# stanfordnlp/mac-network

Hardware: AMD Instinct MI355X
Metric: questions/sec fwd+bwd (B=64,d=512,p=12,KB=14x14x1024) at 1/2/4/8 MI355X (higher is better)
Workload: dtype f32 (3xfp16-split emulation); 1 GPU

## Files before the change

### mac-network_amd/csrc/macx_wgrad_h2.hip.h

```cpp
#pragma once
#include "macx_gemm_tn.hip.h"
#include "macx_h2.hip.h"

namespace macx {

__device__ __forceinline__ float sum16_h2(float v) {
  v += __shfl_xor(v, 1, 64);
  v += __shfl_xor(v, 2, 64);
  v += __shfl_xor(v, 4, 64);
  v += __shfl_xor(v, 8, 64);
  return v;
}
__device__ __forceinline__ uint32_t pk_mul_f16(uint32_t a, uint32_t b) {
  return __builtin_bit_cast(uint32_t, __builtin_bit_cast(f16x2_t, a) * __builtin_bit_cast(f16x2_t, b));
}
__device__ __forceinline__ uint32_t pk_pow2_f16(int k) {
  const float f = k < -30 ? 0.f : h2_pow2(k);
  return pk_f16(f, f);
}

struct ReadAttBwdH2P {
  int B, N, d;
  const float* att;
  const float* da;
  H2View I2;
  const float* c;
  const float* wk;
  int act;
  const uint8_t* bytes;
  float inv_keep;
  H2View dI2;
  float* dc;
  float* dwk_part;
  float* db2_part;
  float* dbk_part;
  const float* dl;
  int no_out;
};

constexpr int RABH_THREADS = 1024;
constexpr int RABH_CHUNK = 128;
__global__ __launch_bounds__(RABH_THREADS) void read_att_bwd_h2_kernel(ReadAttBwdH2P p) {
  __shared__ float s_dl[1024];
  __shared__ float s_red[RABH_THREADS / 64];
  __shared__ float s_mx[16][RABH_CHUNK];
  const int b = blockIdx.x, slab = blockIdx.y;
  const int tid = threadIdx.x, lane = tid & 63;
  const int wave = __builtin_amdgcn_readfirstlane(tid >> 6);
  constexpr int NWV = RABH_THREADS / 64;
  if (p.dl) {
    for (int n = tid; n < p.N; n += RABH_THREADS) s_dl[n] = p.dl[(size_t)b * p.N + n];
    __syncthreads();
  } else {
  float dot = 0.f;
  for (int n = tid; n < p.N; n += RABH_THREADS) dot += p.att[(size_t)b * p.N + n] * p.da[(size_t)b * p.N + n];
  dot = wave_sum(dot);
  if (lane == 0) s_red[wave] = dot;
  __syncthreads();
  dot = 0.f;
#pragma unroll
  for (int w = 0; w < NWV; ++w) dot += s_red[w];
  __syncthreads();
  float dls = 0.f;
  for (int n = tid; n < p.N; n += RABH_THREADS) {
    const float dl = p.att[(size_t)b * p.N + n] * (p.da[(size_t)b * p.N + n] - dot);
    s_dl[n] = dl;
    dls += dl;
  }
  dls = wave_sum(dls);
  if (lane == 0) s_red[wave] = dls;
  __syncthreads();
  if (tid == 0 && slab == 0) {
    float t = 0.f;
#pragma unroll
    for (int w = 0; w < NWV; ++w) t += s_red[w];
    p.dbk_part[b] = t;
  }
  }

  const int kg = slab * 16 + wave;
  const int col0 = slab * 128 + wave * 8;
  float cv[8], wv[8];
  {
    const f32x4 c0 = *reinterpret_cast<const f32x4*>(p.c + (size_t)b * p.d + col0), c1 = *reinterpret_cast<const f32x4*>(p.c + (size_t)b * p.d + col0 + 4);
    const f32x4 w0 = *reinterpret_cast<const f32x4*>(p.wk + col0), w1 = *reinterpret_cast<const f32x4*>(p.wk + col0 + 4);
#pragma unroll
    for (int e = 0; e < 4; ++e) { cv[e] = c0[e]; cv[4 + e] = c1[e]; wv[e] = w0[e]; wv[4 + e] = w1[e]; }
  }
  const size_t iRp = p.I2.Rp(), oRp = p.dI2.Rp();
  const char* i0 = p.I2.plane(0);
  const size_t ipb = p.I2.plane_bytes(), opb = p.dI2.plane_bytes();
  char* o0 = p.dI2.plane(0);
  const int icb = p.I2.cb(), ocb = p.dI2.cb();
  float a_dc[8], a_dw[8], a_db[8];
#pragma unroll
  for (int e = 0; e < 8; ++e) a_dc[e] = a_dw[e] = a_db[e] = 0.f;

  auto rows = [&](auto act_c) {
    constexpr int ACT = decltype(act_c)::value;
    for (int n0 = 0; n0 < p.N; n0 += RABH_CHUNK) {
      float o[RABH_CHUNK / 64][8];
#pragma unroll
      for (int j = 0; j < RABH_CHUNK / 64; ++j) {
        const int lrow = lane + 64 * j, n = n0 + lrow;
        float m = 0.f;
        if (n < p.N) {
          const size_t row = (size_t)b * p.N + n;
          const char* src = i0 + ((size_t)kg * iRp + row) * 16;
          float i2[8];
          h2_join8(*reinterpret_cast<const u32x4*>(src), *reinterpret_cast<const u32x4*>(src + ipb),
                   h2_pow2(-(int)p.I2.exps()[row * icb + slab]), i2);
          const float dl = s_dl[n];
          const uint32_t bits = p.bytes ? (uint32_t)p.bytes[(size_t)kg * iRp + row] : 0xFFu;
#pragma unroll
          for (int e = 0; e < 8; ++e) {
            const float zv = i2[e] * cv[e];
            const float g = act_apply(ACT, zv);
            const float f = ((bits >> e) & 1u) ? p.inv_keep : 0.f;
            const float dz = (dl * wv[e]) * f * act_grad_from_out(ACT, g);
            const float ov = dz * cv[e];
            o[j][e] = ov;
            a_dw[e] = fmaf(dl, g * f, a_dw[e]);
            a_dc[e] = fmaf(dz, i2[e], a_dc[e]);
            a_db[e] += ov;
            m = fmaxf(m, fabsf(ov));
          }
        }
        s_mx[wave][lrow] = m;
      }
      if (p.no_out) continue;
      __syncthreads();
#pragma unroll
      for (int j = 0; j < RABH_CHUNK / 64; ++j) {
        const int lrow = lane + 64 * j, n = n0 + lrow;
        if (n < p.N) {
          float m = s_mx[0][lrow];
#pragma unroll
          for (int k = 1; k < 16; ++k) m = fmaxf(m, s_mx[k][lrow]);
          const int ex = h2_exponent(m);
          const float sc = h2_pow2(ex);
          float xs[8];
#pragma unroll
          for (int e = 0; e < 8; ++e) xs[e] = o[j][e] * sc;
          u32x4 hi, lo;
          h2_split8(xs, hi, lo);
          const size_t row = (size_t)b * p.N + n;
          char* dst = o0 + ((size_t)kg * oRp + row) * 16;
          *reinterpret_cast<u32x4*>(dst) = hi;
          *reinterpret_cast<u32x4*>(dst + opb) = lo;
          if (wave == 0) p.dI2.exps()[row * ocb + slab] = (int8_t)ex;
        }
      }
      __syncthreads();
    }
  };
  switch (p.act) {
    case ACT_TANH: rows(std::integral_constant<int, ACT_TANH>{}); break;
    case ACT_SIGMOID: rows(std::integral_constant<int, ACT_SIGMOID>{}); break;
    case ACT_ELU: rows(std::integral_constant<int, ACT_ELU>{}); break;
    case ACT_RELU: rows(std::integral_constant<int, ACT_RELU>{}); break;
    default: rows(std::integral_constant<int, ACT_NON>{}); break;
  }
#pragma unroll
  for (int e = 0; e < 8; ++e) {
    a_dc[e] = wave_sum(a_dc[e]);
    a_dw[e] = wave_sum(a_dw[e]);
    a_db[e] = wave_sum(a_db[e]);
  }
  if (lane == 0) {
    float* dc = p.dc + (size_t)b * p.d + col0;
#pragma unroll
    for (int e = 0; e < 8; ++e) {
      dc[e] += a_dc[e];
      p.dwk_part[(size_t)b * p.d + col0 + e] = a_dw[e];
      p.db2_part[(size_t)b * p.d + col0 + e] = a_db[e];
    }
  }
}

struct TnH2P {
  int M;
  int Kd, Jd;
  int nsplit, rows_per_split;
  int R;
  const char* A; size_t a_stride; int a_mod;
  const char* G; size_t g_stride;
  const int* ecomA;
  const int* ecomG;
  int ecom_nb;
  uint16_t* ftab;
  float* part;
  int dbg;
};
__host__ __device__ inline size_t wgrad_h2_mpad(size_t M) { return (M + 63) & ~(size_t)31; }

typedef short s16x4 __attribute__((ext_vector_type(4)));
__device__ __forceinline__ u32x2 tr_read(const char* lds_addr) {
  const s16x4 v = __builtin_amdgcn_ds_read_tr16_b64_v4i16((__attribute__((address_space(3))) s16x4*)lds_addr);
  return __builtin_bit_cast(u32x2, v);
}

constexpr int WH_APL = 8 * 2 * 512;
template <int KW, int JW> constexpr int wh_stage_bytes() { return 2 * (KW + JW) * WH_APL + 256; }
template <int KW, int JW> constexpr int wh_ring() { return KW + JW == 4 ? 2 : (KW + JW == 3 ? 3 : 4); }

__global__ __launch_bounds__(256) void wgrad_h2_factors_kernel(TnH2P p0, TnH2P p1) {
  const TnH2P& p = blockIdx.y ? p1 : p0;
  __shared__ int sE[2][8];
  if (threadIdx.x < 16) {
    const int w = threadIdx.x >> 3, k = threadIdx.x & 7;
    sE[w][k] = h2_emin_final(w ? p.ecomG : p.ecomA, p.ecom_nb, k);
  }
  __syncthreads();
  const size_t mpad = wgrad_h2_mpad((size_t)p.M);
  const size_t m = (size_t)blockIdx.x * 256 + threadIdx.x;
  if (m >= mpad) return;
  const int acb = p.Kd >> 7, gcb = p.Jd >> 7;
  const H2View a0{const_cast<char*>(p.A), p.R, p.Kd}, g0{const_cast<char*>(p.G), p.R, p.Jd};
  if (m >= (size_t)p.M) {
    for (int i = 0; i < acb * gcb; ++i) p.ftab[(size_t)i * mpad + m] = 0;
    return;
  }
  const int ti = (int)(m / p.R), rr = (int)(m - (size_t)ti * p.R);
  const int ar = p.a_mod ? (int)(m % p.a_mod) : rr;
  const int8_t* ea = reinterpret_cast<const int8_t*>(p.A + (p.a_mod ? 0 : (size_t)ti * p.a_stride) + 2 * a0.plane_bytes()) + (size_t)ar * acb;
  const int8_t* eg = reinterpret_cast<const int8_t*>(p.G + (size_t)ti * p.g_stride + 2 * g0.plane_bytes()) + (size_t)rr * gcb;
  for (int k = 0; k < acb; ++k) {
    const int da = sE[0][k] - (int)ea[k];
    for (int j = 0; j < gcb; ++j)
      p.ftab[((size_t)k * gcb + j) * mpad + m] = (uint16_t)(pk_pow2_f16(da + sE[1][j] - (int)eg[j]) & 0xFFFFu);
  }
}

__device__ __forceinline__ void dma4b(const char* g, char* lds_wave_base) {
  const uint32_t l = __builtin_amdgcn_readfirstlane(
      (uint32_t)(uintptr_t)(__attribute__((address_space(3))) char*)lds_wave_base);
  asm volatile("s_mov_b32 m0, %1\n\ts_nop 0\n\tglobal_load_lds_dword %0, off" ::"v"(g), "s"(l) : "memory", "m0");
}

inline int wgrad_pipe_mode() { const int v = tune_get(MACX_TUNE_WGRAD_PIPE, 3); return (v >= 0 && v <= 3) ? v : 3; }

template <int KW, int JW, int PIPE = 0>
__global__ __launch_bounds__(512) void wgrad_h2_kernel(TnH2P p0, TnH2P p1) {
  const TnH2P& p = blockIdx.y ? p1 : p0;
  extern __shared__ __attribute__((aligned(16))) float smem[];
  char* lds = reinterpret_cast<char*>(smem);
  constexpr int KT = KW * T_TILE;
  constexpr int JT = JW * T_TILE;
  constexpr int APL = KW * WH_APL;
  constexpr int GPL = JW * WH_APL;
  constexpr int DATA = 2 * APL + 2 * GPL;
  constexpr int STAGE = wh_stage_bytes<KW, JW>();
  constexpr int RING = wh_ring<KW, JW>();
  constexpr int NI = 2 * (KW + JW);
  constexpr int NR = 4 * KW;
  constexpr int NC = 2 * JW;

  const int ntj = p.Jd / JT;
  const int ntk = p.Kd / KT;
  const int ntile = ntj * ntk;
  const int nblk = gridDim.x;
  int v = blockIdx.x;
  if ((nblk & 7) == 0) v = (blockIdx.x & 7) * (nblk >> 3) + (blockIdx.x >> 3);
  const int split = v / ntile;
  const int tile = v % ntile;
  const int tk = tile / ntj, tj = tile % ntj;

  const int tid = threadIdx.x, lane = tid & 63;
  const int wave = __builtin_amdgcn_readfirstlane(tid >> 6);
  const int wr = wave >> 2, wc = wave & 3;
  const int aq = KW == 2 ? wr : 0;
  const int gq = JW == 2 ? (wc >> 1) : 0;
  const int m_begin = split * p.rows_per_split;
  const int m_end = min(p.M, m_begin + p.rows_per_split);
  const int nchunk = (m_end - m_begin + 31) >> 5;

  const H2View a0{const_cast<char*>(p.A), p.R, p.Kd}, g0{const_cast<char*>(p.G), p.R, p.Jd};
  const size_t Rp = a0.Rp();
  const size_t apb = a0.plane_bytes(), gpb = g0.plane_bytes();
  const int gcb = g0.cb();
  const size_t mpad = wgrad_h2_mpad((size_t)p.M);

  f32x4 acc[NR][NC];
#pragma unroll
  for (int t = 0; t < NR; ++t)
#pragma unroll
    for (int c = 0; c < NC; ++c) acc[t][c] = f32x4{0.f, 0.f, 0.f, 0.f};

  const int sl_m = (lane >> 5) * 16 + ((lane & 31) >> 1), sl_kg = lane & 1;
  const int ft_t = lane < 16 * KW * JW ? (lane >> 4) : 0;
  const uint16_t* ft_src = p.ftab + ((size_t)(tk * KW + ft_t / JW) * gcb + tj * JW + ft_t % JW) * mpad + (lane < 16 * KW * JW ? (lane & 15) * 2 : 0);
  auto issue = [&](int s_raw) __attribute__((always_inline)) {
    const int ch = min(s_raw, nchunk - 1);
    const int m0 = m_begin + ch * 32;
    const int mc = min(m0 + sl_m, p.M - 1);
    const int ti = mc / p.R, rr = mc - ti * p.R;
    const int ar = p.a_mod ? (mc % p.a_mod) : rr;
    const char* ab = p.A + (p.a_mod ? 0 : (size_t)ti * p.a_stride);
    const char* gb = p.G + (size_t)ti * p.g_stride;
    char* st = lds + (s_raw % RING) * STAGE;
#pragma unroll
    for (int j = 0; j < NI; ++j) {
      const int u = wave * NI + j;
      if (u < 16 * KW) {
        const int pl = u / (8 * KW), ct = u - pl * 8 * KW;
        dma16b(ab + pl * apb + ((size_t)(tk * 16 * KW + 2 * ct + sl_kg) * Rp + ar) * 16, st + pl * APL + ct * 1024);
      } else {
        const int ug = u - 16 * KW;
        const int pl = ug / (8 * JW), ct = ug - pl * 8 * JW;
        dma16b(gb + pl * gpb + ((size_t)(tj * 16 * JW + 2 * ct + sl_kg) * Rp + rr) * 16, st + 2 * APL + pl * GPL + ct * 1024);
      }
    }
    if (wave == 0) dma4b(reinterpret_cast<const char*>(ft_src + m0), st + DATA);
  };
  auto issue_part = [&](int s_raw, int part) __attribute__((always_inline)) {
    static_assert(!PIPE || (KW == 2 && JW == 2), "the split issue assumes waves 0-3 stage A and waves 4-7 stage G");
    const int ch = min(s_raw, nchunk - 1);
    const int m0 = m_begin + ch * 32;
    const int mc = min(m0 + sl_m, p.M - 1);
    const int ti = mc / p.R, rr = mc - ti * p.R;
    char* st = lds + (s_raw % RING) * STAGE;
    if (part == 1) {
      if (wave < 4) {
        const int ar = p.a_mod ? (mc % p.a_mod) : rr;
        const char* ab = p.A + (p.a_mod ? 0 : (size_t)ti * p.a_stride);
#pragma unroll
        for (int j = 0; j < NI; ++j) {
          const int u = wave * NI + j;
          const int pl = u / (8 * KW), ct = u - pl * 8 * KW;
          dma16b(ab + pl * apb + ((size_t)(tk * 16 * KW + 2 * ct + sl_kg) * Rp + ar) * 16, st + pl * APL + ct * 1024);
        }
      }
    } else {
      if (wave >= 4) {
        const char* gb = p.G + (size_t)ti * p.g_stride;
#pragma unroll
        for (int j = 0; j < NI; ++j) {
          const int ug = wave * NI + j - 16 * KW;
          const int pl = ug / (8 * JW), ct = ug - pl * 8 * JW;
          dma16b(gb + pl * gpb + ((size_t)(tj * 16 * JW + 2 * ct + sl_kg) * Rp + rr) * 16, st + 2 * APL + pl * GPL + ct * 1024);
        }
      }
      if (wave == 0) dma4b(reinterpret_cast<const char*>(ft_src + m0), st + DATA);
    }
  };
  auto frag = [&](const char* tile) __attribute__((always_inline)) {
    const u32x2 lo = tr_read(tile + lane * 8), hi = tr_read(tile + 512 + lane * 8);
    return u32x4{lo[0], lo[1], hi[0], hi[1]};
  };
  auto compute = [&](int buf) __attribute__((always_inline)) {
    const char* sa = lds + buf * STAGE + (wr * NR) * 1024;
    const char* sg = lds + buf * STAGE + 2 * APL + (wc * NC) * 1024;
    const uint16_t* ft = reinterpret_cast<const uint16_t*>(lds + buf * STAGE + DATA) + (aq * JW + gq) * 32 + (lane >> 4) * 4;
    const u32x2 f0 = *reinterpret_cast<const u32x2*>(ft), f1 = *reinterpret_cast<const u32x2*>(ft + 16);
    u32x4 gf[2][NC];
#pragma unroll
    for (int pl = 0; pl < 2; ++pl)
#pragma unroll
      for (int c = 0; c < NC; ++c) {
        u32x4 w = frag(sg + pl * GPL + c * 1024);
        w[0] = pk_mul_f16(w[0], f0[0]); w[1] = pk_mul_f16(w[1], f0[1]);
        w[2] = pk_mul_f16(w[2], f1[0]); w[3] = pk_mul_f16(w[3], f1[1]);
        gf[pl][c] = w;
      }
#pragma unroll
    for (int ap = 1; ap >= 0; --ap) {
      u32x4 af[NR];
#pragma unroll
      for (int t = 0; t < NR; ++t) af[t] = frag(sa + ap * APL + t * 1024);
#pragma unroll
      for (int bp = 1 - ap; bp >= 0; --bp)
#pragma unroll
        for (int t = 0; t < NR; ++t)
#pragma unroll
          for (int c = 0; c < NC; ++c) acc[t][c] = mfma_f16(af[t], gf[bp][c], acc[t][c]);
    }
  };

  if constexpr (PIPE) {
    if (nchunk > 0) {
      const int my_n = NI + (wave == 0 ? 1 : 0);
      issue(0);
      issue(1);
      wait_vmcnt_n(my_n);
      __syncthreads();
#pragma unroll 1
      for (int s = 0; s < nchunk; ++s) {
        const int buf = s & 1;
        const char* sa = lds + buf * STAGE + (wr * NR) * 1024;
        const char* sg = lds + buf * STAGE + 2 * APL + (wc * NC) * 1024;
        const uint16_t* ft = reinterpret_cast<const uint16_t*>(lds + buf * STAGE + DATA) + (aq * JW + gq) * 32 + (lane >> 4) * 4;
        const u32x2 f0 = *reinterpret_cast<const u32x2*>(ft), f1 = *reinterpret_cast<const u32x2*>(ft + 16);
        u32x4 gf[2][NC];
#pragma unroll
        for (int pl = 0; pl < 2; ++pl)
#pragma unroll
          for (int c = 0; c < NC; ++c) {
            u32x4 w = frag(sg + pl * GPL + c * 1024);
            w[0] = pk_mul_f16(w[0], f0[0]); w[1] = pk_mul_f16(w[1], f0[1]);
            w[2] = pk_mul_f16(w[2], f1[0]); w[3] = pk_mul_f16(w[3], f1[1]);
            gf[pl][c] = w;
          }
        __syncthreads();
        if (!(p.dbg & 2048)) issue_part(s + 2, 0);
        u32x4 af[NR];
#pragma unroll
        for (int t = 0; t < NR; ++t) af[t] = frag(sa + APL + t * 1024);
        if (!(p.dbg & 1024)) {
#pragma unroll
          for (int t = 0; t < NR; ++t)
#pragma unroll
            for (int c = 0; c < NC; ++c) acc[t][c] = mfma_f16(af[t], gf[0][c], acc[t][c]);
        }
#pragma unroll
        for (int t = 0; t < NR; ++t) af[t] = frag(sa + t * 1024);
        __syncthreads();
        if (!(p.dbg & 2048)) issue_part(s + 2, 1);
        if (!(p.dbg & 1024)) {
#pragma unroll
          for (int bp = 1; bp >= 0; --bp)
#pragma unroll
            for (int t = 0; t < NR; ++t)
#pragma unroll
              for (int c = 0; c < NC; ++c) acc[t][c] = mfma_f16(af[t], gf[bp][c], acc[t][c]);
        }
        if (p.dbg & 2048) wait_vmcnt<0>(); else wait_vmcnt_n(my_n);
        __syncthreads();
      }
      wait_vmcnt<0>();
    }
  } else
  if (nchunk > 0) {
    const int my_n = (NI + (wave == 0 ? 1 : 0)) * (RING - 2);
#pragma unroll
    for (int s = 0; s < RING - 1; ++s) issue(s);
    wait_vmcnt_n(my_n);
    __syncthreads();
#pragma unroll 1
    for (int s = 0; s < nchunk; ++s) {
      if (!(p.dbg & 2048)) issue(s + RING - 1);
      if (!(p.dbg & 1024)) compute(s % RING);
      wait_vmcnt_n(my_n);
      __syncthreads();
    }
    wait_vmcnt<0>();
  }

  __syncthreads();

  const float sc = h2_unscale(h2_emin_final(p.ecomA, p.ecom_nb, tk * KW + aq), h2_emin_final(p.ecomG, p.ecom_nb, tj * JW + gq));
  float* out = p.part + (size_t)split * p.Kd * p.Jd + (size_t)(tk * KT + wr * 16 * NR) * p.Jd + tj * JT + wc * 32 * JW;
  constexpr int CW = 32 * JW, LDW = CW + 4;
  constexpr int LPR = CW / 4, RPI = 64 / LPR;
  float* tw = reinterpret_cast<float*>(lds) + wave * (32 * LDW);
#pragma unroll
  for (int tp = 0; tp < NR; tp += 2) {
#pragma unroll
    for (int u = 0; u < 2; ++u)
#pragma unroll
      for (int c = 0; c < NC; ++c)
#pragma unroll
        for (int e = 0; e < 4; ++e) tw[(u * 16 + (lane >> 4) * 4 + e) * LDW + c * 16 + (lane & 15)] = acc[tp + u][c][e] * sc;
#pragma unroll
    for (int i = 0; i < 32 / RPI; ++i) {
      const int r = i * RPI + lane / LPR, c4 = (lane % LPR) * 4;
      f32x4* dst = reinterpret_cast<f32x4*>(out + (size_t)(tp * 16 + r) * p.Jd + c4);
      f32x4 val = *reinterpret_cast<const f32x4*>(tw + r * LDW + c4);
      *dst = val;
    }
  }
}

inline int wgrad_h2_jw(int Jd) { return (Jd % 256 == 0) ? 2 : 1; }
inline int wgrad_h2_kw(int Kd) { return (Kd % 256 == 0) ? 2 : 1; }
inline int wgrad_h2_tiles(int Kd, int Jd) { return (Kd / (wgrad_h2_kw(Kd) * T_TILE)) * (Jd / (wgrad_h2_jw(Jd) * T_TILE)); }

template <int KW, int JW, int PIPE = 0>
inline hipError_t wgrad_h2_launch_t(const TnH2P& p, hipStream_t st) {
  auto kern = wgrad_h2_kernel<KW, JW, PIPE>;
  constexpr size_t lds = (size_t)wh_ring<KW, JW>() * wh_stage_bytes<KW, JW>();
  hipError_t e = lds_attr_once(reinterpret_cast<const void*>(kern), lds);
  if (e != hipSuccess) return e;
  const int grid = wgrad_h2_tiles(p.Kd, p.Jd) * p.nsplit;
  hipLaunchKernelGGL(kern, dim3(grid), dim3(512), lds, st, p, p);
  return hipGetLastError();
}
inline hipError_t wgrad_h2_launch(const TnH2P& p, hipStream_t st);
inline hipError_t wgrad_h2_launch_pair(const TnH2P& a, const TnH2P& b, hipStream_t st) {
  const bool same = a.M == b.M && a.Kd == b.Kd && a.Jd == b.Jd && a.nsplit == b.nsplit && a.rows_per_split == b.rows_per_split && a.R == b.R;
  if (!(same && wgrad_pipe_mode() >= 2 && wgrad_h2_kw(a.Kd) == 2 && wgrad_h2_jw(a.Jd) == 2 && a.ftab != b.ftab && a.part != b.part)) {
    hipError_t e = wgrad_h2_launch(a, st);
    return e != hipSuccess ? e : wgrad_h2_launch(b, st);
  }
  if (a.rows_per_split % 32 != 0 || !a.ftab || !b.ftab) return hipErrorInvalidValue;
  const size_t mpad = wgrad_h2_mpad((size_t)a.M);
  hipLaunchKernelGGL(wgrad_h2_factors_kernel, dim3((unsigned)((mpad + 255) / 256), 2), dim3(256), 0, st, a, b);
  hipError_t e = hipGetLastError();
  if (e != hipSuccess) return e;
  auto kern = wgrad_h2_kernel<2, 2, 1>;
  constexpr size_t lds = (size_t)wh_ring<2, 2>() * wh_stage_bytes<2, 2>();
  e = lds_attr_once(reinterpret_cast<const void*>(kern), lds);
  if (e != hipSuccess) return e;
  hipLaunchKernelGGL(kern, dim3(wgrad_h2_tiles(a.Kd, a.Jd) * a.nsplit, 2), dim3(512), lds, st, a, b);
  return hipGetLastError();
}
inline hipError_t wgrad_h2_launch(const TnH2P& p, hipStream_t st) {
  if (p.rows_per_split % 32 != 0 || !p.ftab) return hipErrorInvalidValue;
  const size_t mpad = wgrad_h2_mpad((size_t)p.M);
  hipLaunchKernelGGL(wgrad_h2_factors_kernel, dim3((unsigned)((mpad + 255) / 256)), dim3(256), 0, st, p, p);
  hipError_t e = hipGetLastError();
  if (e != hipSuccess) return e;
  const int kw = wgrad_h2_kw(p.Kd), jw = wgrad_h2_jw(p.Jd);
  if (kw == 2 && jw == 2) return wgrad_pipe_mode() ? wgrad_h2_launch_t<2, 2, 1>(p, st) : wgrad_h2_launch_t<2, 2, 0>(p, st);
  if (kw == 2) return wgrad_h2_launch_t<2, 1>(p, st);
  return jw == 2 ? wgrad_h2_launch_t<1, 2>(p, st) : wgrad_h2_launch_t<1, 1>(p, st);
}

struct SbH2P {
  int B, N, d;
  int qpg;
  H2View X;
  H2View dI1;
  const float* y;
  const float* W1a;
  float* dW1a_part;
  float* dW1b_part;
  float* dy_part;
  int nsteps;
  size_t x_step, g_step, y_step;
  int dbg;
};

constexpr int SBH_STAGE = 4 * WH_APL;
constexpr int SBH_CW = 8;
constexpr int SBH_MAXROWS = 4096;
constexpr int SBH_RING = 4;
constexpr int SBH_MAXQ = 32;

template <bool DY>
__global__ __launch_bounds__(512) void sb_h2_kernel(SbH2P p) {
  extern __shared__ __attribute__((aligned(16))) float smem[];
  char* lds = reinterpret_cast<char*>(smem);
  uint16_t* ftab = reinterpret_cast<uint16_t*>(lds + SBH_RING * SBH_STAGE);
  float* ytab = reinterpret_cast<float*>(lds + SBH_RING * SBH_STAGE + SBH_MAXROWS * 2);
  float* sctab = ytab + SBH_MAXQ * T_TILE;
  int* qmn = reinterpret_cast<int*>(sctab + SBH_MAXQ);

  const int nt = p.d / T_TILE;
  const int ntile = nt * nt;
  const int nblk = gridDim.x;
  int v = blockIdx.x;
  if ((nblk & 7) == 0) v = (blockIdx.x & 7) * (nblk >> 3) + (blockIdx.x >> 3);
  const int group = v / ntile;
  const int tile = v % ntile;
  const int tk = tile / nt, tj = tile % nt;

  const int tid = threadIdx.x, lane = tid & 63;
  const int wave = __builtin_amdgcn_readfirstlane(tid >> 6);
  const int wr = wave >> 2, wc = wave & 3;

  const int nchunk = (p.N + 31) >> 5;
  const int b_begin = group * p.qpg;
  const int b_end = min(p.B, b_begin + p.qpg);
  const int nq = b_end - b_begin;
  const int total = nq * nchunk;
  const size_t Rp = p.X.Rp();
  const size_t xpb = p.X.plane_bytes(), gpb = p.dI1.plane_bytes();
  const int xcb = p.X.cb(), gcb = p.dI1.cb();
  H2View vX = p.X, vG = p.dI1;
  const float* yS = p.y;
  const int rows_q = nchunk * 32;

  const int sl_half = lane >> 5, sl_row = (lane & 31) >> 1, sl_kg = lane & 1;
  const int sl_m = sl_half * 16 + sl_row;
  auto issue = [&](int s_raw) __attribute__((always_inline)) {
    const int s = min(s_raw, total - 1);
    const int qi = s / nchunk, ch = s - qi * nchunk;
    const int n = min(ch * 32 + sl_m, p.N - 1);
    const size_t row = (size_t)(b_begin + qi) * p.N + n;
    char* st = lds + (s_raw % SBH_RING) * SBH_STAGE;
#pragma unroll
    for (int j = 0; j < 4; ++j) {
      const int u = wave * 4 + j;
      const int im = u >> 3, ct = u & 7;
      const char* src = (im < 2 ? vX.base + (im & 1) * xpb + ((size_t)(tk * 16 + 2 * ct + sl_kg) * Rp + row) * 16
                                : vG.base + (im & 1) * gpb + ((size_t)(tj * 16 + 2 * ct + sl_kg) * Rp + row) * 16);
      dma16b(src, st + im * WH_APL + ct * 1024);
    }
  };
  auto tables = [&]() __attribute__((always_inline)) {
  if (tid < 2 * SBH_MAXQ) qmn[tid] = 127;
  __syncthreads();
  for (int i0 = 0; i0 < nq * rows_q; i0 += 512) {
    const int i = i0 + tid;
    const int qi = i / rows_q, n = i - qi * rows_q;
    int ex = 127, eg = 127;
    if (i < nq * rows_q && n < p.N) {
      const size_t row = (size_t)(b_begin + qi) * p.N + n;
      ex = (int)vX.exps()[row * xcb + tk];
      eg = (int)vG.exps()[row * gcb + tj];
    }
    const int q_lo = min(i0 + (tid & ~63), nq * rows_q - 1) / rows_q, q_hi = min(i0 + (tid | 63), nq * rows_q - 1) / rows_q;
    for (int q = q_lo; q <= q_hi; ++q) {
      int mx = qi == q ? ex : 127, mg = qi == q ? eg : 127;
#pragma unroll
      for (int o = 32; o > 0; o >>= 1) { mx = min(mx, __shfl_xor(mx, o, 64)); mg = min(mg, __shfl_xor(mg, o, 64)); }
      if (lane == 0) { atomicMin(qmn + q, mx); atomicMin(qmn + SBH_MAXQ + q, mg); }
    }
  }
  __syncthreads();
  for (int i = tid; i < nq * rows_q; i += 512) {
    const int qi = i / rows_q, n = i - qi * rows_q;
    const int b = b_begin + qi;
    uint16_t f = 0;
    if (n < p.N) {
      const size_t row = (size_t)b * p.N + n;
      const int k = (min(qmn[qi], 126) - (int)vX.exps()[row * xcb + tk]) + (min(qmn[SBH_MAXQ + qi], 126) - (int)vG.exps()[row * gcb + tj]);
      f = (uint16_t)(pk_pow2_f16(k) & 0xFFFFu);
    }
    ftab[i] = f;
  }
  for (int i = tid; i < nq * T_TILE; i += 512)
    ytab[i] = yS[(size_t)(b_begin + (i >> 7)) * p.d + tk * T_TILE + (i & 127)];
  if (tid < nq) sctab[tid] = h2_unscale(min(qmn[tid], 126), min(qmn[SBH_MAXQ + tid], 126));
  };

  f32x4 accS[4][2], accA[4][2], accB[4][2];
#pragma unroll
  for (int t = 0; t < 4; ++t)
#pragma unroll
    for (int c = 0; c < 2; ++c) accS[t][c] = accA[t][c] = accB[t][c] = f32x4{0.f, 0.f, 0.f, 0.f};

  auto frag = [&](const char* tile) __attribute__((always_inline)) {
    const u32x2 lo = tr_read(tile + lane * 8), hi = tr_read(tile + 512 + lane * 8);
    return u32x4{lo[0], lo[1], hi[0], hi[1]};
  };
  auto compute = [&](int buf, int qi, int ch) __attribute__((always_inline)) {
    const char* sa = lds + buf * SBH_STAGE + (wr * 4) * 1024;
    const char* sg = lds + buf * SBH_STAGE + 2 * WH_APL + (wc * 2) * 1024;
    const uint16_t* ft = ftab + qi * rows_q + ch * 32 + (lane >> 4) * 4;
    const u32x2 f0 = *reinterpret_cast<const u32x2*>(ft), f1 = *reinterpret_cast<const u32x2*>(ft + 16);
    u32x4 gf[2][2];
#pragma unroll
    for (int pl = 0; pl < 2; ++pl)
#pragma unroll
      for (int c = 0; c < 2; ++c) {
        u32x4 w = frag(sg + pl * WH_APL + c * 1024);
        w[0] = pk_mul_f16(w[0], f0[0]); w[1] = pk_mul_f16(w[1], f0[1]);
        w[2] = pk_mul_f16(w[2], f1[0]); w[3] = pk_mul_f16(w[3], f1[1]);
        gf[pl][c] = w;
      }
#pragma unroll
    for (int ap = 1; ap >= 0; --ap) {
      u32x4 af[4];
#pragma unroll
      for (int t = 0; t < 4; ++t) af[t] = frag(sa + ap * WH_APL + t * 1024);
#pragma unroll
      for (int bp = 1 - ap; bp >= 0; --bp)
#pragma unroll
        for (int t = 0; t < 4; ++t)
#pragma unroll
          for (int c = 0; c < 2; ++c) accS[t][c] = mfma_f16(af[t], gf[bp][c], accS[t][c]);
    }
  };
  float w1[4][4][2];
  if (DY) {
    const float* wb = p.W1a + (size_t)(tk * T_TILE + wr * 64 + (lane >> 4) * 4) * p.d + tj * T_TILE + wc * 32 + (lane & 15);
#pragma unroll
    for (int t = 0; t < 4; ++t)
#pragma unroll
      for (int e = 0; e < 4; ++e)
#pragma unroll
        for (int c = 0; c < 2; ++c) w1[t][e][c] = wb[(size_t)(t * 16 + e) * p.d + c * 16];
#pragma unroll
    for (int t = 0; t < 4; ++t)
#pragma unroll
      for (int e = 0; e < 4; ++e)
#pragma unroll
        for (int c = 0; c < 2; ++c) asm volatile("" : "+v"(w1[t][e][c]));
  }
  auto consume = [&](int b) __attribute__((always_inline)) {
    const float sc = sctab[b - b_begin];
    f32x4 y4[4];
#pragma unroll
    for (int t = 0; t < 4; ++t) y4[t] = *reinterpret_cast<const f32x4*>(ytab + (b - b_begin) * T_TILE + wr * 64 + t * 16 + (lane >> 4) * 4);
#pragma unroll
    for (int t = 0; t < 4; ++t)
#pragma unroll
      for (int e = 0; e < 4; ++e) {
        const int k = tk * T_TILE + wr * 64 + t * 16 + (lane >> 4) * 4 + e;
        const float yk = y4[t][e];
        float dyp = 0.f;
#pragma unroll
        for (int c = 0; c < 2; ++c) {
          const float sv = accS[t][c][e] * sc;
          accB[t][c][e] += sv;
          accA[t][c][e] = fmaf(yk, sv, accA[t][c][e]);
          if (DY) dyp = fmaf(w1[t][e][c], sv, dyp);
          accS[t][c][e] = 0.f;
        }
        if (DY) {
          dyp = sum16_h2(dyp);
          if ((lane & 15) == 0) p.dy_part[((size_t)(tj * 4 + wc) * p.B + b) * p.d + k] = dyp;
        }
      }
  };

#pragma unroll 1
  for (int step = 0; step < p.nsteps; ++step) {
  vX.base = p.X.base + (size_t)step * p.x_step; vG.base = p.dI1.base + (size_t)step * p.g_step;
  yS = p.y + (size_t)step * p.y_step;
  if (total > 0) {
    issue(0);
    issue(1);
    issue(2);
  }
  tables();
  if (total > 0) {
    wait_vmcnt<8>();
    __syncthreads();
    int qi = 0, qch = 0;
#pragma unroll 1
    for (int s = 0; s < total; ++s) {
      if (!(p.dbg & 2048)) issue(s + 3);
      if (!(p.dbg & 1024)) compute(s % SBH_RING, qi, qch);
      wait_vmcnt<8>();
      if (++qch == nchunk) {
        if (!(p.dbg & 512)) consume(b_begin + qi);
        qch = 0; ++qi;
      }
      __syncthreads();
    }
    wait_vmcnt<0>();
  }
  __syncthreads();
  }

  float* oa = p.dW1a_part + (size_t)group * p.d * p.d;
  float* ob = p.dW1b_part + (size_t)group * p.d * p.d;
  constexpr int LDW = 36;
  float* tw = reinterpret_cast<float*>(lds) + wave * (64 * LDW);
#pragma unroll
  for (int which = 0; which < 2; ++which) {
#pragma unroll
    for (int t = 0; t < 4; ++t)
#pragma unroll
      for (int c = 0; c < 2; ++c)
#pragma unroll
        for (int e = 0; e < 4; ++e)
          tw[(t * 16 + (lane >> 4) * 4 + e) * LDW + c * 16 + (lane & 15)] = which ? accB[t][c][e] : accA[t][c][e];
    float* o = (which ? ob : oa) + (size_t)(tk * T_TILE + wr * 64) * p.d + tj * T_TILE + wc * 32;
#pragma unroll
    for (int i = 0; i < 8; ++i) {
      const int r = i * 8 + (lane >> 3), c4 = (lane & 7) * 4;
      *reinterpret_cast<f32x4*>(o + (size_t)r * p.d + c4) = *reinterpret_cast<const f32x4*>(tw + r * LDW + c4);
    }
  }
}

constexpr int SBW_STAGE = 2 * WH_APL + 4 * WH_APL;
constexpr int SBW_RING = 3;
constexpr int SBW_MAXQ = 4;
constexpr int SBW_MAXROWS = 1024;

constexpr int SBW_TABLES = SBW_MAXROWS * 2 + SBW_MAXQ * T_TILE * 4 + 4 * SBW_MAXQ * 4;
template <bool CONT>
__global__ __launch_bounds__(512) void sb_h2w_kernel(SbH2P p) {
  extern __shared__ __attribute__((aligned(16))) float smem[];
  char* lds = reinterpret_cast<char*>(smem);
  char* tab0 = lds + SBW_RING * SBW_STAGE;
  uint16_t* ftab = reinterpret_cast<uint16_t*>(tab0);
  float* ytab = reinterpret_cast<float*>(tab0 + SBW_MAXROWS * 2);
  int* qmn = reinterpret_cast<int*>(ytab + SBW_MAXQ * T_TILE);
  float* yold = reinterpret_cast<float*>(tab0 + (CONT ? 2 : 1) * SBW_TABLES);

  const int ntk = p.d / T_TILE, ntj = p.d / (2 * T_TILE);
  const int ntile = ntk * ntj;
  const int nblk = gridDim.x;
  int v = blockIdx.x;
  if ((nblk & 7) == 0) v = (blockIdx.x & 7) * (nblk >> 3) + (blockIdx.x >> 3);
  const int group = v / ntile;
  const int tile = v % ntile;
  const int tk = tile / ntj, tj = tile % ntj;

  const int tid = threadIdx.x, lane = tid & 63;
  const int wave = __builtin_amdgcn_readfirstlane(tid >> 6);
  const int wr = wave >> 2, wc = wave & 3;
  const int gq = wc >> 1;

  const int nchunk = (p.N + 31) >> 5;
  const int b_begin = group * p.qpg;
  const int b_end = min(p.B, b_begin + p.qpg);
  const int nq = b_end - b_begin;
  const int total = nq * nchunk;
  const size_t Rp = p.X.Rp();
  const size_t xpb = p.X.plane_bytes(), gpb = p.dI1.plane_bytes();
  const int xcb = p.X.cb(), gcb = p.dI1.cb();
  H2View vX = p.X, vG = p.dI1;
  const float* yS = p.y;
  const int rows_q = nchunk * 32;

  const int sl_half = lane >> 5, sl_row = (lane & 31) >> 1, sl_kg = lane & 1;
  const int sl_m = sl_half * 16 + sl_row;
  const uint32_t lds0 = lds_addr_of(lds);
  auto issue = [&](int s_raw) __attribute__((always_inline)) {
    const int s = min(s_raw, total - 1);
    const int qi = s / nchunk, ch = s - qi * nchunk;
    const int n = min(ch * 32 + sl_m, p.N - 1);
    const uint32_t voff = (uint32_t)(((size_t)sl_kg * Rp + (size_t)(b_begin + qi) * p.N + n) * 16);
    const uint32_t st = lds0 + (uint32_t)((s_raw % SBW_RING) * SBW_STAGE);
#pragma unroll
    for (int j = 0; j < 2; ++j) {
      const int u = wave * 2 + j, pl = u >> 3, ct = u & 7;
      dma16b_s(vX.base + pl * xpb + (size_t)(tk * 16 + 2 * ct) * Rp * 16, voff, st + pl * WH_APL + ct * 1024);
    }
#pragma unroll
    for (int j = 0; j < 4; ++j) {
      const int u = wave * 4 + j, pl = u >> 4, ct = u & 15;
      dma16b_s(vG.base + pl * gpb + (size_t)(tj * 32 + 2 * ct) * Rp * 16, voff, st + 2 * WH_APL + pl * 2 * WH_APL + ct * 1024);
    }
  };
  uint16_t* ftab_c = ftab;
  float* ytab_c = ytab;
  int* qmn_c = qmn;
  auto tables = [&]() __attribute__((always_inline)) {
    if (tid < 3 * SBW_MAXQ) qmn[tid] = 127;
    __syncthreads();
    for (int i0 = 0; i0 < nq * rows_q; i0 += 512) {
      const int i = i0 + tid;
      const int qi = i / rows_q, n = i - qi * rows_q;
      int ex = 127, eg0 = 127, eg1 = 127;
      if (i < nq * rows_q && n < p.N) {
        const size_t row = (size_t)(b_begin + qi) * p.N + n;
        ex = (int)vX.exps()[row * xcb + tk];
        eg0 = (int)vG.exps()[row * gcb + 2 * tj];
        eg1 = (int)vG.exps()[row * gcb + 2 * tj + 1];
      }
      const int q_lo = min(i0 + (tid & ~63), nq * rows_q - 1) / rows_q, q_hi = min(i0 + (tid | 63), nq * rows_q - 1) / rows_q;
      for (int q = q_lo; q <= q_hi; ++q) {
        int mx = qi == q ? ex : 127, mg = qi == q ? min(eg0, eg1) : 127;
#pragma unroll
        for (int o = 32; o > 0; o >>= 1) { mx = min(mx, __shfl_xor(mx, o, 64)); mg = min(mg, __shfl_xor(mg, o, 64)); }
        if (lane == 0) { atomicMin(qmn + q, mx); atomicMin(qmn + SBW_MAXQ + q, mg); }
      }
    }
    __syncthreads();
    for (int i = tid; i < 2 * nq * rows_q; i += 512) {
      const int blk = i / (nq * rows_q), r = i - blk * nq * rows_q;
      const int qi = r / rows_q, n = r - qi * rows_q;
      uint16_t f = 0;
      if (n < p.N) {
        const size_t row = (size_t)(b_begin + qi) * p.N + n;
        const int k = (min(qmn[qi], 126) - (int)vX.exps()[row * xcb + tk]) + (min(qmn[SBW_MAXQ + qi], 126) - (int)vG.exps()[row * gcb + 2 * tj + blk]);
        f = (uint16_t)(pk_pow2_f16(k) & 0xFFFFu);
      }
      ftab[blk * (SBW_MAXROWS / 2) + r] = f;
    }
    for (int i = tid; i < nq * T_TILE; i += 512)
      ytab[i] = yS[(size_t)(b_begin + (i >> 7)) * p.d + tk * T_TILE + (i & 127)];
  };

  f32x4 accT[4][4], accA[4][4];
#pragma unroll
  for (int t = 0; t < 4; ++t)
#pragma unroll
    for (int c = 0; c < 4; ++c) accT[t][c] = accA[t][c] = f32x4{0.f, 0.f, 0.f, 0.f};

  auto frag = [&](const char* tile) __attribute__((always_inline)) {
    const u32x2 lo = tr_read(tile + lane * 8), hi = tr_read(tile + 512 + lane * 8);
    return u32x4{lo[0], lo[1], hi[0], hi[1]};
  };
  auto compute = [&](int buf, int qi, int ch) __attribute__((always_inline)) {
    const char* sa = lds + buf * SBW_STAGE + (wr * 4) * 1024;
    const char* sg = lds + buf * SBW_STAGE + 2 * WH_APL + (wc * 4) * 1024;
    const uint16_t* ft = ftab_c + gq * (SBW_MAXROWS / 2) + qi * rows_q + ch * 32 + (lane >> 4) * 4;
    const u32x2 f0 = *reinterpret_cast<const u32x2*>(ft), f1 = *reinterpret_cast<const u32x2*>(ft + 16);
    u32x4 gf[2][4];
#pragma unroll
    for (int pl = 0; pl < 2; ++pl)
#pragma unroll
      for (int c = 0; c < 4; ++c) {
        u32x4 w = frag(sg + pl * 2 * WH_APL + c * 1024);
        w[0] = pk_mul_f16(w[0], f0[0]); w[1] = pk_mul_f16(w[1], f0[1]);
        w[2] = pk_mul_f16(w[2], f1[0]); w[3] = pk_mul_f16(w[3], f1[1]);
        gf[pl][c] = w;
      }
#pragma unroll
    for (int ap = 1; ap >= 0; --ap) {
      u32x4 af[4];
#pragma unroll
      for (int t = 0; t < 4; ++t) af[t] = frag(sa + ap * WH_APL + t * 1024);
#pragma unroll
      for (int bp = 1 - ap; bp >= 0; --bp)
#pragma unroll
        for (int t = 0; t < 4; ++t)
#pragma unroll
          for (int c = 0; c < 4; ++c) accT[t][c] = mfma_f16(af[t], gf[bp][c], accT[t][c]);
    }
  };
  int ex_prev = 0, eg_prev = 0, ybuf = 0;
  bool pending = false;
  auto keep_y = [&](const float* ynext) __attribute__((always_inline)) {
    if (tid < T_TILE) yold[(ybuf ^ 1) * T_TILE + tid] = ynext ? ynext[tid] : 0.f;
    ybuf ^= 1;
  };
  auto fold = [&](const float* ynext, int ex_next, int eg_next) __attribute__((always_inline)) {
    const float sc = h2_unscale(ex_prev, eg_prev);
    const float mv = h2_pow2(max(min((ex_next + eg_next) - (ex_prev + eg_prev), 126), -126));
    const float* yp = yold + ybuf * T_TILE;
#pragma unroll
    for (int t = 0; t < 4; ++t) {
      const int k0 = wr * 64 + t * 16 + (lane >> 4) * 4;
      f32x4 yn = f32x4{0.f, 0.f, 0.f, 0.f};
      if (ynext) yn = *reinterpret_cast<const f32x4*>(ynext + k0);
      const f32x4 yo = *reinterpret_cast<const f32x4*>(yp + k0);
#pragma unroll
      for (int e = 0; e < 4; ++e) {
        const float dy = (yo[e] - yn[e]) * sc;
#pragma unroll
        for (int c = 0; c < 4; ++c) {
          accA[t][c][e] = fmaf(dy, accT[t][c][e], accA[t][c][e]);
          accT[t][c][e] *= mv;
        }
      }
    }
    keep_y(ynext);
    ex_prev = ex_next; eg_prev = eg_next;
  };

  if constexpr (CONT) {
    const int G = p.nsteps * total;
    auto issue_g = [&](int g_raw) __attribute__((always_inline)) {
      const int g = min(g_raw, G - 1);
      const int ist = g / total, sg = g - ist * total;
      const int qi = sg / nchunk, ch = sg - qi * nchunk;
      const int n = min(ch * 32 + sl_m, p.N - 1);
      const uint32_t voff = (uint32_t)(((size_t)sl_kg * Rp + (size_t)(b_begin + qi) * p.N + n) * 16);
      const uint32_t st = lds0 + (uint32_t)((g_raw % SBW_RING) * SBW_STAGE);
      const char* xb = p.X.base + (size_t)ist * p.x_step;
      const char* gb = p.dI1.base + (size_t)ist * p.g_step;
#pragma unroll
      for (int j = 0; j < 2; ++j) {
        const int u = wave * 2 + j, pl = u >> 3, ct = u & 7;
        dma16b_s(xb + pl * xpb + (size_t)(tk * 16 + 2 * ct) * Rp * 16, voff, st + pl * WH_APL + ct * 1024);
      }
#pragma unroll
      for (int j = 0; j < 4; ++j) {
        const int u = wave * 4 + j, pl = u >> 4, ct = u & 15;
        dma16b_s(gb + pl * gpb + (size_t)(tj * 32 + 2 * ct) * Rp * 16, voff, st + 2 * WH_APL + pl * 2 * WH_APL + ct * 1024);
      }
    };
    issue_g(0);
    issue_g(1);
    tables();
    wait_vmcnt<6>();
    __syncthreads();
    const int nrows = nq * rows_q;
    const int t_q = min(tid, nrows - 1) / rows_q, t_n = min(tid, nrows - 1) - t_q * rows_q;
    const bool t_row = tid < nrows && t_n < p.N;
    const size_t t_grow = (size_t)(b_begin + t_q) * p.N + min(t_n, p.N - 1);
    const bool t_yv = tid < nq * T_TILE;
    const size_t t_yoff = (size_t)(b_begin + (t_yv ? (tid >> 7) : 0)) * p.d + tk * T_TILE + (tid & 127);
    int t_ex = 127, t_g0 = 127, t_g1 = 127;
    float t_y = 0.f;
    int step = 0, sg = 0, qi = 0, qch = 0;
#pragma unroll 1
    for (int g = 0; g < G; ++g) {
      const bool more = step + 1 < p.nsteps;
      char* nset = tab0 + ((step + 1) & 1) * SBW_TABLES;
      uint16_t* ftab_n = reinterpret_cast<uint16_t*>(nset);
      float* ytab_n = reinterpret_cast<float*>(nset + SBW_MAXROWS * 2);
      int* qmn_n = reinterpret_cast<int*>(ytab_n + SBW_MAXQ * T_TILE);
      if (more && sg == 1) {
        const H2View nX{const_cast<char*>(p.X.base) + (size_t)(step + 1) * p.x_step, p.X.R, p.X.C};
        const H2View nG{const_cast<char*>(p.dI1.base) + (size_t)(step + 1) * p.g_step, p.dI1.R, p.dI1.C};
        const int8_t* ax = nX.exps() + t_grow * xcb + tk;
        const int8_t* ag = nG.exps() + t_grow * gcb + 2 * tj;
        const float* ay = p.y + (size_t)(step + 1) * p.y_step + t_yoff;
        asm volatile("global_load_sbyte %0, %1, off" : "=v"(t_ex) : "v"(ax) : "memory");
        asm volatile("global_load_sbyte %0, %1, off" : "=v"(t_g0) : "v"(ag) : "memory");
        asm volatile("global_load_sbyte %0, %1, off offset:1" : "=v"(t_g1) : "v"(ag) : "memory");
        asm volatile("global_load_dword %0, %1, off" : "=v"(t_y) : "v"(ay) : "memory");
      }
      if (!(p.dbg & 2048)) issue_g(g + 2);
      if (qch == 0) {
        const float* yn = ytab_c + qi * T_TILE;
        const int exn = min(qmn_c[qi], 126), egn = min(qmn_c[SBW_MAXQ + qi], 126);
        if (pending) {
          if (!(p.dbg & 512)) fold(yn, exn, egn);
        } else {
          keep_y(yn);
          ex_prev = exn; eg_prev = egn;
          pending = true;
        }
      }
      if (!(p.dbg & 1024)) compute(g % SBW_RING, qi, qch);
      if (p.dbg & 2048) wait_vmcnt<0>(); else wait_vmcnt<6>();
      if (more) {
        if (sg == 0) {
          if (tid < 3 * SBW_MAXQ) qmn_n[tid] = 127;
        } else if (sg == 1) {
          asm volatile("" : "+v"(t_ex), "+v"(t_g0), "+v"(t_g1), "+v"(t_y));
          if (!t_row) { t_ex = 127; t_g0 = 127; t_g1 = 127; }
          const int q_lo = min(tid & ~63, nrows - 1) / rows_q, q_hi = min(tid | 63, nrows - 1) / rows_q;
          for (int q = q_lo; q <= q_hi; ++q) {
            int mx = t_q == q ? t_ex : 127, mg = t_q == q ? min(t_g0, t_g1) : 127;
#pragma unroll
            for (int o = 32; o > 0; o >>= 1) { mx = min(mx, __shfl_xor(mx, o, 64)); mg = min(mg, __shfl_xor(mg, o, 64)); }
            if (lane == 0) { atomicMin(qmn_n + q, mx); atomicMin(qmn_n + SBW_MAXQ + q, mg); }
          }
        } else if (sg == 2) {
          if (tid < nrows) {
            const int bx = min(qmn_n[t_q], 126), bg = min(qmn_n[SBW_MAXQ + t_q], 126);
            ftab_n[tid] = t_row ? (uint16_t)(pk_pow2_f16((bx - t_ex) + (bg - t_g0)) & 0xFFFFu) : (uint16_t)0;
            ftab_n[(SBW_MAXROWS / 2) + tid] = t_row ? (uint16_t)(pk_pow2_f16((bx - t_ex) + (bg - t_g1)) & 0xFFFFu) : (uint16_t)0;
          }
          if (t_yv) ytab_n[tid] = t_y;
        }
      }
      if (++qch == nchunk) { qch = 0; ++qi; }
      if (++sg == total) {
        sg = 0; qi = 0; ++step;
        char* cset = tab0 + (step & 1) * SBW_TABLES;
        ftab_c = reinterpret_cast<uint16_t*>(cset);
        ytab_c = reinterpret_cast<float*>(cset + SBW_MAXROWS * 2);
        qmn_c = reinterpret_cast<int*>(ytab_c + SBW_MAXQ * T_TILE);
      }
      __syncthreads();
    }
    wait_vmcnt<0>();
    __syncthreads();
  } else {
#pragma unroll 1
  for (int step = 0; step < p.nsteps; ++step) {
    vX.base = p.X.base + (size_t)step * p.x_step; vG.base = p.dI1.base + (size_t)step * p.g_step;
    yS = p.y + (size_t)step * p.y_step;
    if (total > 0) { issue(0); issue(1); }
    tables();
    if (total > 0) {
      wait_vmcnt<6>();
      __syncthreads();
      int qi = 0, qch = 0;
#pragma unroll 1
      for (int s = 0; s < total; ++s) {
        if (!(p.dbg & 2048)) issue(s + 2);
        if (qch == 0) {
          const float* yn = ytab + qi * T_TILE;
          const int exn = min(qmn[qi], 126), egn = min(qmn[SBW_MAXQ + qi], 126);
          if (pending) {
            if (!(p.dbg & 512)) fold(yn, exn, egn);
          } else {
            keep_y(yn);
            ex_prev = exn; eg_prev = egn;
            pending = true;
          }
        }
        if (!(p.dbg & 1024)) compute(s % SBW_RING, qi, qch);
        wait_vmcnt<6>();
        if (++qch == nchunk) { qch = 0; ++qi; }
        __syncthreads();
      }
      wait_vmcnt<0>();
    }
    __syncthreads();
  }
  }
  if (pending && !(p.dbg & 512)) fold(nullptr, ex_prev, eg_prev);
  const float scT = h2_unscale(ex_prev, eg_prev);

  float* oa = p.dW1a_part + (size_t)group * p.d * p.d;
  float* ob = p.dW1b_part + (size_t)group * p.d * p.d;
  constexpr int LDW = 68;
  float* tw = reinterpret_cast<float*>(lds) + wave * (64 * LDW);
#pragma unroll
  for (int which = 0; which < 2; ++which) {
#pragma unroll
    for (int t = 0; t < 4; ++t)
#pragma unroll
      for (int c = 0; c < 4; ++c)
#pragma unroll
        for (int e = 0; e < 4; ++e)
          tw[(t * 16 + (lane >> 4) * 4 + e) * LDW + c * 16 + (lane & 15)] = which ? accT[t][c][e] * scT : accA[t][c][e];
    float* o = (which ? ob : oa) + (size_t)(tk * T_TILE + wr * 64) * p.d + tj * 2 * T_TILE + wc * 64;
#pragma unroll
    for (int i = 0; i < 16; ++i) {
      const int r = i * 4 + (lane >> 4), c4 = (lane & 15) * 4;
      *reinterpret_cast<f32x4*>(o + (size_t)r * p.d + c4) = *reinterpret_cast<const f32x4*>(tw + r * LDW + c4);
    }
  }
}

inline bool sb_h2_wide_ok(int B, int N, int d) { return d % 256 == 0 && B >= 1 && N >= 1 && ((N + 31) / 32) * 32 <= SBW_MAXROWS / 2; }
inline int sb_h2_wide_qpg(int B, int N, int d) {
  const int tiles = (d / 128) * (d / 256);
  int groups = 256 / tiles;
  if (groups < 1) groups = 1;
  int qpg = (B + groups - 1) / groups;
  const int rows_q = ((N + 31) / 32) * 32;
  const int cap = min(SBW_MAXQ, (SBW_MAXROWS / 2) / rows_q);
  if (qpg > cap) qpg = cap;
  return qpg < 1 ? 1 : qpg;
}
inline int sb_cont_mode() { return tune_get(MACX_TUNE_SB_CONT, 1); }
inline hipError_t sb_h2w_launch(const SbH2P& p, hipStream_t st) {
  const int nchunk = (p.N + 31) >> 5;
  if (p.qpg < 1 || p.qpg > SBW_MAXQ || p.qpg * nchunk * 32 > SBW_MAXROWS / 2 || p.d % 256 || p.dy_part || p.nsteps < 1) return hipErrorInvalidValue;
  const int ngroup = (p.B + p.qpg - 1) / p.qpg;
  const bool cont = sb_cont_mode() && p.nsteps > 1 && nchunk >= 3 && p.qpg * nchunk * 32 <= 512;
  if (cont) {
    constexpr size_t lds = (size_t)SBW_RING * SBW_STAGE + 2 * SBW_TABLES + 2 * T_TILE * 4;
    static_assert(lds <= 160 * 1024, "two table sets fit beside the ring");
    hipError_t e = lds_attr_once(reinterpret_cast<const void*>(sb_h2w_kernel<true>), lds);
    if (e != hipSuccess) return e;
    hipLaunchKernelGGL(sb_h2w_kernel<true>, dim3((p.d / 128) * (p.d / 256) * ngroup), dim3(512), lds, st, p);
    return hipGetLastError();
  }
  constexpr size_t lds = (size_t)SBW_RING * SBW_STAGE + SBW_TABLES + 2 * T_TILE * 4;
  hipError_t e = lds_attr_once(reinterpret_cast<const void*>(sb_h2w_kernel<false>), lds);
  if (e != hipSuccess) return e;
  hipLaunchKernelGGL(sb_h2w_kernel<false>, dim3((p.d / 128) * (p.d / 256) * ngroup), dim3(512), lds, st, p);
  return hipGetLastError();
}

inline hipError_t sb_h2_launch(const SbH2P& p, hipStream_t st) {
  const int nchunk = (p.N + 31) >> 5;
  if (p.qpg * nchunk * 32 > SBH_MAXROWS || p.qpg > SBH_MAXQ) return hipErrorInvalidValue;
  constexpr size_t lds = SBH_RING * SBH_STAGE + SBH_MAXROWS * 2 + SBH_MAXQ * T_TILE * 4 + SBH_MAXQ * 4 + 2 * SBH_MAXQ * 4;
  if (p.nsteps < 1 || (p.nsteps > 1 && p.dy_part)) return hipErrorInvalidValue;
  auto kern = p.dy_part ? sb_h2_kernel<true> : sb_h2_kernel<false>;
  hipError_t e = lds_attr_once(reinterpret_cast<const void*>(kern), lds);
  if (e != hipSuccess) return e;
  const int nt = p.d / T_TILE;
  const int ngroup = (p.B + p.qpg - 1) / p.qpg;
  hipLaunchKernelGGL(kern, dim3(nt * nt * ngroup), dim3(512), lds, st, p);
  return hipGetLastError();
}

}
```

Before: 18430 questions/s.

## Carry the hi*hi split product into the next stage to overlap LDS reads

Adds a CARRY variant of the continuous weight-gradient kernel that splits each stage's LDS fragment reads into two halves. The xh*gh MFMA block of one stage is deferred and issued at the start of the next stage, while that stage's first-half reads are in flight. The goal is to hide LDS latency and the barrier/table work behind matrix-core work. The variant becomes the default through the tune mode (default 2). It costs more live registers for the carried fragments, which risks occupancy loss or spills. It also reorders the fp16-split accumulation.

```diff
diff --git a/mac-network_amd/csrc/macx_wgrad_h2.hip.h b/mac-network_amd/csrc/macx_wgrad_h2.hip.h
--- a/mac-network_amd/csrc/macx_wgrad_h2.hip.h
+++ b/mac-network_amd/csrc/macx_wgrad_h2.hip.h
@@ -764,8 +764,9 @@
 constexpr int SBW_MAXROWS = 1024;
 
 constexpr int SBW_TABLES = SBW_MAXROWS * 2 + SBW_MAXQ * T_TILE * 4 + 4 * SBW_MAXQ * 4;
-template <bool CONT>
+template <bool CONT, bool CARRY = false>
 __global__ __launch_bounds__(512) void sb_h2w_kernel(SbH2P p) {
+  static_assert(CONT || !CARRY, "the carried term is a form of the continuous stage stream");
   extern __shared__ __attribute__((aligned(16))) float smem[];
   char* lds = reinterpret_cast<char*>(smem);
   char* tab0 = lds + SBW_RING * SBW_STAGE;
@@ -897,6 +898,49 @@
 #pragma unroll
           for (int c = 0; c < 4; ++c) accT[t][c] = mfma_f16(af[t], gf[bp][c], accT[t][c]);
     }
+  };
+  struct StageFrags { u32x4 gh[4], gl[4], xl[4], xh[4]; u32x2 f0, f1; };
+  u32x4 cx[4], cg[4];
+  auto stage_reads = [&](int buf, int qi, int ch, int half, StageFrags& r) __attribute__((always_inline)) {
+    const char* sa = lds + buf * SBW_STAGE + (wr * 4) * 1024;
+    const char* sg = lds + buf * SBW_STAGE + 2 * WH_APL + (wc * 4) * 1024;
+    if (half == 0) {
+      const uint16_t* ft = ftab_c + gq * (SBW_MAXROWS / 2) + qi * rows_q + ch * 32 + (lane >> 4) * 4;
+      r.f0 = *reinterpret_cast<const u32x2*>(ft); r.f1 = *reinterpret_cast<const u32x2*>(ft + 16);
+#pragma unroll
+      for (int c = 0; c < 4; ++c) r.gh[c] = frag(sg + c * 1024);
+    } else {
+#pragma unroll
+      for (int t = 0; t < 4; ++t) r.xl[t] = frag(sa + WH_APL + t * 1024);
+#pragma unroll
+      for (int c = 0; c < 4; ++c) r.gl[c] = frag(sg + 2 * WH_APL + c * 1024);
+#pragma unroll
+      for (int t = 0; t < 4; ++t) r.xh[t] = frag(sa + t * 1024);
+    }
+  };
+  auto head = [&](StageFrags& r) __attribute__((always_inline)) {
+    auto scale = [&](u32x4& w) __attribute__((always_inline)) {
+      w[0] = pk_mul_f16(w[0], r.f0[0]); w[1] = pk_mul_f16(w[1], r.f0[1]);
+      w[2] = pk_mul_f16(w[2], r.f1[0]); w[3] = pk_mul_f16(w[3], r.f1[1]);
+    };
+#pragma unroll
+    for (int c = 0; c < 4; ++c) { scale(r.gh[c]); scale(r.gl[c]); }
+#pragma unroll
+    for (int t = 0; t < 4; ++t)
+#pragma unroll
+      for (int c = 0; c < 4; ++c) accT[t][c] = mfma_f16(r.xl[t], r.gh[c], accT[t][c]);
+#pragma unroll
+    for (int t = 0; t < 4; ++t)
+#pragma unroll
+      for (int c = 0; c < 4; ++c) accT[t][c] = mfma_f16(r.xh[t], r.gl[c], accT[t][c]);
+#pragma unroll
+    for (int i = 0; i < 4; ++i) { cx[i] = r.xh[i]; cg[i] = r.gh[i]; }
+  };
+  auto carried = [&]() __attribute__((always_inline)) {
+#pragma unroll
+    for (int t = 0; t < 4; ++t)
+#pragma unroll
+      for (int c = 0; c < 4; ++c) accT[t][c] = mfma_f16(cx[t], cg[c], accT[t][c]);
   };
   int ex_prev = 0, eg_prev = 0, ybuf = 0;
   bool pending = false;
@@ -982,6 +1026,14 @@
         asm volatile("global_load_sbyte %0, %1, off offset:1" : "=v"(t_g1) : "v"(ag) : "memory");
         asm volatile("global_load_dword %0, %1, off" : "=v"(t_y) : "v"(ay) : "memory");
       }
+      StageFrags fr;
+      if constexpr (CARRY) {
+        if (!(p.dbg & 1024)) {
+          stage_reads(g % SBW_RING, qi, qch, 0, fr);
+          if (g > 0) carried();
+        }
+        __builtin_amdgcn_sched_barrier(0);
+      }
       if (!(p.dbg & 2048)) issue_g(g + 2);
       if (qch == 0) {
         const float* yn = ytab_c + qi * T_TILE;
@@ -994,7 +1046,14 @@
           pending = true;
         }
       }
-      if (!(p.dbg & 1024)) compute(g % SBW_RING, qi, qch);
+      if constexpr (CARRY) {
+        if (!(p.dbg & 1024)) {
+          stage_reads(g % SBW_RING, qi, qch, 1, fr);
+          head(fr);
+        }
+      } else {
+        if (!(p.dbg & 1024)) compute(g % SBW_RING, qi, qch);
+      }
       if (p.dbg & 2048) wait_vmcnt<0>(); else wait_vmcnt<6>();
       if (more) {
         if (sg == 0) {
@@ -1027,6 +1086,9 @@
         qmn_c = reinterpret_cast<int*>(ytab_c + SBW_MAXQ * T_TILE);
       }
       __syncthreads();
+    }
+    if constexpr (CARRY) {
+      if (!(p.dbg & 1024)) carried();
     }
     wait_vmcnt<0>();
     __syncthreads();
@@ -1101,7 +1163,7 @@
   if (qpg > cap) qpg = cap;
   return qpg < 1 ? 1 : qpg;
 }
-inline int sb_cont_mode() { return tune_get(MACX_TUNE_SB_CONT, 1); }
+inline int sb_cont_mode() { const int v = tune_get(MACX_TUNE_SB_CONT, 2); return (v >= 0 && v <= 2) ? v : 2; }
 inline hipError_t sb_h2w_launch(const SbH2P& p, hipStream_t st) {
   const int nchunk = (p.N + 31) >> 5;
   if (p.qpg < 1 || p.qpg > SBW_MAXQ || p.qpg * nchunk * 32 > SBW_MAXROWS / 2 || p.d % 256 || p.dy_part || p.nsteps < 1) return hipErrorInvalidValue;
@@ -1110,9 +1172,10 @@
   if (cont) {
     constexpr size_t lds = (size_t)SBW_RING * SBW_STAGE + 2 * SBW_TABLES + 2 * T_TILE * 4;
     static_assert(lds <= 160 * 1024, "two table sets fit beside the ring");
-    hipError_t e = lds_attr_once(reinterpret_cast<const void*>(sb_h2w_kernel<true>), lds);
+    auto kern = sb_cont_mode() == 2 ? sb_h2w_kernel<true, true> : sb_h2w_kernel<true, false>;
+    hipError_t e = lds_attr_once(reinterpret_cast<const void*>(kern), lds);
     if (e != hipSuccess) return e;
-    hipLaunchKernelGGL(sb_h2w_kernel<true>, dim3((p.d / 128) * (p.d / 256) * ngroup), dim3(512), lds, st, p);
+    hipLaunchKernelGGL(kern, dim3((p.d / 128) * (p.d / 256) * ngroup), dim3(512), lds, st, p);
     return hipGetLastError();
   }
   constexpr size_t lds = (size_t)SBW_RING * SBW_STAGE + SBW_TABLES + 2 * T_TILE * 4;
```

Measured after the change: 18470 questions/s, median of 6. No clear change (+0.2%).
